# yangt1013/SPEINet

Measured on AMD Instinct MI355X. Metric: deblurred 720p frames/sec, higher is better.
Workload: dtype f16 (correlation top2)

## Files before the change

### speinet_amd/csrc/conv32_ws16.hip

```cpp
#include "common.h"

namespace {

constexpr int C = 32, KS = 5, PAD = 2, NTAP = KS * KS;
constexpr int TH = 16, TW = 32;
constexpr int IH = TH + KS - 1, IW = TW + KS - 1;
constexpr int PITCH = 2 * C + 16;
constexpr int SLAB = IH * IW * PITCH;
constexpr int NTHR = 256, RT = 4;

struct WsParams {
    const void* a;
    const void* wfrag;
    const float* bias;
    void* out;
    int H, W, batch, act;
    int tiles_x, tiles_y, total;
    long long* stamps;
};

__device__ __forceinline__ void mfma_aw(f32x16& acc, const lpv<_Float16>::x8& w, const lpv<_Float16>::x8& b) {
    asm volatile("v_mfma_f32_32x32x16_f16 %0, %1, %2, %0" : "+v"(acc) : "a"(w), "v"(b));
}
__device__ __forceinline__ void mfma_aw(f32x16& acc, const lpv<__bf16>::x8& w, const lpv<__bf16>::x8& b) {
    asm volatile("v_mfma_f32_32x32x16_bf16 %0, %1, %2, %0" : "+v"(acc) : "a"(w), "v"(b));
}

template <typename TA> struct Chunk { static constexpr int CPP = sizeof(TA) == 4 ? 8 : 4; };

template <typename LP, typename TA, typename TO>
__global__ __launch_bounds__(NTHR, 1) void conv32_ws_kernel(const WsParams p) {
    typedef typename lpv<LP>::x8 lp8;
    typedef typename lpv<LP>::x4 lp4;
    constexpr int CPP = Chunk<TA>::CPP;
    constexpr int NCH = IH * IW * CPP;
    constexpr int NIT = (NCH + NTHR - 1) / NTHR;
    constexpr int NPH = sizeof(TA) == 4 ? 2 : 1;
    constexpr int NITH = (NIT + NPH - 1) / NPH;
    extern __shared__ __attribute__((aligned(16))) unsigned char smem[];

    const int tid = threadIdx.x, lane = tid & 63, wave = tid >> 6;
    const int fr = lane & 31, fk = lane >> 5;

    lp8 wreg[NTAP][2];
    {
        const LP* wp = static_cast<const LP*>(p.wfrag) + lane * 8;
#pragma unroll
        for (int t = 0; t < NTAP; ++t)
#pragma unroll
            for (int s = 0; s < 2; ++s) wreg[t][s] = *reinterpret_cast<const lp8*>(wp + (t * 2 + s) * 512);
    }
    float biasv[16];
#pragma unroll
    for (int r = 0; r < 16; ++r) biasv[r] = p.bias ? p.bias[8 * (r >> 2) + 4 * fk + (r & 3)] : 0.f;

    typedef u32x4 stage_t;
    stage_t sreg[NITH];
    const size_t map_elems = (size_t)p.H * p.W * C;
    const int per_map = p.tiles_x * p.tiles_y;

    auto tile_origin = [&](int t, int& b, int& oy0, int& ox0) {
        b = t / per_map;
        const int r = t - b * per_map;
        const int ty = r / p.tiles_x;
        oy0 = ty * TH;
        ox0 = (r - ty * p.tiles_x) * TW;
    };
    constexpr int PPI = NTHR / CPP, E = 16 / (int)sizeof(TA);
    const int p0 = tid / CPP, sub = tid - p0 * CPP;
    const int iy0 = p0 / IW, ix0 = p0 - iy0 * IW;
    const int lds0 = p0 * PITCH + sub * (sizeof(TA) == 4 ? 8 : 16);
    auto advance = [](int& iy, int& ix) {
        ix += PPI % IW;
        iy += PPI / IW;
        if (ix >= IW) { ix -= IW; ++iy; }
    };
    auto load_slab = [&](int t, int ph) {
        int b, oy0, ox0;
        tile_origin(t, b, oy0, ox0);
        const TA* base = static_cast<const TA*>(p.a) + (size_t)b * map_elems + sub * E;
        int iy = iy0, ix = ix0;
#pragma unroll
        for (int it = 0; it < NIT; ++it) {
            if (it >= ph * NITH && it < (ph + 1) * NITH) {
                const int iyc = min(iy, IH - 1);
                const int gy = min(max(oy0 - PAD + iyc, 0), p.H - 1), gx = min(max(ox0 - PAD + ix, 0), p.W - 1);
                sreg[it - ph * NITH] = *reinterpret_cast<const stage_t*>(base + (gy * p.W + gx) * C);
            }
            advance(iy, ix);
        }
    };
    auto store_slab = [&](int t, int buf, int ph, int lo, int hi) {
        int b, oy0, ox0;
        tile_origin(t, b, oy0, ox0);
        unsigned char* sl = smem + buf * SLAB + lds0;
        int iy = iy0, ix = ix0;
#pragma unroll
        for (int it = 0; it < NIT; ++it) {
            if (it >= ph * NITH + lo && it < ph * NITH + hi && it < (ph + 1) * NITH && iy < IH) {
                const int j = it - ph * NITH;
                const bool ok = ((unsigned)(oy0 - PAD + iy) < (unsigned)p.H) & ((unsigned)(ox0 - PAD + ix) < (unsigned)p.W);
                if constexpr (sizeof(TA) == 4) {
                    const f32x4 v = __builtin_bit_cast(f32x4, sreg[j]);
                    lp4 h = to_lp4<LP>(v);
                    if (!ok) h = lp4{(LP)0.f, (LP)0.f, (LP)0.f, (LP)0.f};
                    *reinterpret_cast<lp4*>(sl + it * PPI * PITCH) = h;
                } else {
                    *reinterpret_cast<stage_t*>(sl + it * PPI * PITCH) = ok ? sreg[j] : stage_t{0u, 0u, 0u, 0u};
                }
            }
            advance(iy, ix);
        }
    };

    int t = blockIdx.x;
    if (t >= p.total) return;
#pragma unroll
    for (int ph = 0; ph < NPH; ++ph) {
        load_slab(t, ph);
        store_slab(t, 0, ph, 0, NITH);
    }
    lds_barrier();

    int boff[RT];
#pragma unroll
    for (int i = 0; i < RT; ++i) boff[i] = ((wave * RT + i) * IW + fr) * PITCH + fk * 16;

    int buf = 0;
    for (; t < p.total; t += gridDim.x, buf ^= 1) {
        const int tn = t + gridDim.x;
        const bool more = tn < p.total;
        const int tl = more ? tn : t;
        const bool st_ = t == (int)blockIdx.x + (int)gridDim.x;
        if (st_) SPEI_STAMP(p.stamps, 0);
        load_slab(tl, 0);
        if (st_) SPEI_STAMP(p.stamps, 1);
        __builtin_amdgcn_sched_barrier(0);

        const unsigned char* sl = smem + buf * SLAB;
        f32x16 acc[RT];
#pragma unroll
        for (int i = 0; i < RT; ++i)
#pragma unroll
            for (int r = 0; r < 16; ++r) acc[i][r] = biasv[r];
        lp8 bq[3][RT];
        auto step_off = [](int step) { const int tap = step >> 1; return ((tap / KS) * IW + (tap % KS)) * PITCH + (step & 1) * 32; };
#pragma unroll
        for (int d = 0; d < 2; ++d)
#pragma unroll
            for (int i = 0; i < RT; ++i) bq[d][i] = *reinterpret_cast<const lp8*>(sl + boff[i] + step_off(d));
#pragma unroll
        for (int step = 0; step < NTAP * 2; ++step) {
            const int tap = step >> 1, s2 = step & 1;
            if (step + 2 < NTAP * 2) {
#pragma unroll
                for (int i = 0; i < RT; ++i) bq[(step + 2) % 3][i] = *reinterpret_cast<const lp8*>(sl + boff[i] + step_off(step + 2));
            }
#pragma unroll
            for (int i = 0; i < RT; ++i) mfma_aw(acc[i], wreg[tap][s2], bq[step % 3][i]);
            if (NPH == 2 && step == NTAP) {
                store_slab(tl, buf ^ 1, 0, 0, NITH);
                load_slab(tl, 1);
            }
            if (NPH == 1 && step >= NTAP && ((step - NTAP) & 1) == 0 && (step - NTAP) / 2 < NITH)
                store_slab(tl, buf ^ 1, 0, (step - NTAP) / 2, (step - NTAP) / 2 + 1);
        }

        if (st_) SPEI_STAMP(p.stamps, 2);
        {
            int b, oy0, ox0;
            tile_origin(t, b, oy0, ox0);
            TO* ob = static_cast<TO*>(p.out) + (size_t)b * map_elems;
            const int ox = ox0 + fr;
#pragma unroll
            for (int i = 0; i < RT; ++i) {
                const int oy = oy0 + wave * RT + i;
                if (oy < p.H && ox < p.W) {
                    TO* o = ob + ((size_t)oy * p.W + ox) * C + 4 * fk;
#pragma unroll
                    for (int g = 0; g < 4; ++g) {
                        f32x4 v = {acc[i][4 * g], acc[i][4 * g + 1], acc[i][4 * g + 2], acc[i][4 * g + 3]};
                        if (p.act == SPEI_ACT_RELU) v = f32x4{fmaxf(v[0], 0.f), fmaxf(v[1], 0.f), fmaxf(v[2], 0.f), fmaxf(v[3], 0.f)};
                        if constexpr (sizeof(TO) == 4) *reinterpret_cast<f32x4*>(o + 8 * g) = v;
                        else *reinterpret_cast<lp4*>(o + 8 * g) = to_lp4<LP>(v);
                    }
                }
            }
        }
        if (st_) SPEI_STAMP(p.stamps, 3);
        if (NPH == 2) store_slab(tl, buf ^ 1, 1, 0, NITH);
        else store_slab(tl, buf ^ 1, 0, (NTAP + 1) / 2, NITH);
        if (st_) SPEI_STAMP(p.stamps, 4);
        lds_barrier();
        if (st_) SPEI_STAMP(p.stamps, 5);
    }
}

template <typename LP>
int launch_ws(const WsParams& p, int a16, int o16, hipStream_t st) {
    const size_t lds = 2 * (size_t)SLAB;
    const int cus = spei_num_cus();
    const dim3 grid(p.total < cus ? p.total : cus);
    if (a16 && o16) {
        ensure_dyn_lds<&conv32_ws_kernel<LP, LP, LP>>(lds);
        hipLaunchKernelGGL((conv32_ws_kernel<LP, LP, LP>), grid, dim3(NTHR), lds, st, p);
    } else if (!a16 && o16) {
        ensure_dyn_lds<&conv32_ws_kernel<LP, float, LP>>(lds);
        hipLaunchKernelGGL((conv32_ws_kernel<LP, float, LP>), grid, dim3(NTHR), lds, st, p);
    } else if (a16 && !o16) {
        ensure_dyn_lds<&conv32_ws_kernel<LP, LP, float>>(lds);
        hipLaunchKernelGGL((conv32_ws_kernel<LP, LP, float>), grid, dim3(NTHR), lds, st, p);
    } else {
        ensure_dyn_lds<&conv32_ws_kernel<LP, float, float>>(lds);
        hipLaunchKernelGGL((conv32_ws_kernel<LP, float, float>), grid, dim3(NTHR), lds, st, p);
    }
    return 0;
}

}

extern "C" int spei_conv32_ws16(int fmt, const void* a, int a_fmt, const void* wfrag, const float* bias, void* out, int out_fmt, int batch,
                                int H, int W, int act, spei_stream_t stream) {
    SPEI_REQUIRE(a && wfrag && out, "spei_conv32_ws16: null pointer");
    SPEI_REQUIRE((fmt == SPEI_BF16 || fmt == SPEI_F16) && (a_fmt == SPEI_F32 || a_fmt == fmt) && (out_fmt == SPEI_F32 || out_fmt == fmt),
                 "spei_conv32_ws16: fmt=%d a_fmt=%d out_fmt=%d", fmt, a_fmt, out_fmt);
    SPEI_REQUIRE(batch >= 1 && H > 0 && W > 0 && (int64_t)batch * cdiv(H, TH) * cdiv(W, TW) < (1ll << 30) && (int64_t)H * W < (1ll << 26),
                 "spei_conv32_ws16: batch=%d of %dx%d", batch, H, W);
    SPEI_REQUIRE(act == SPEI_ACT_NONE || act == SPEI_ACT_RELU, "spei_conv32_ws16: act=%d", act);
    SPEI_REQUIRE(((uintptr_t)a | (uintptr_t)wfrag | (uintptr_t)out) % 16 == 0 && a != out, "spei_conv32_ws16: 16-byte alignment, out must not be the input");
    WsParams p;
    p.a = a; p.wfrag = wfrag; p.bias = bias; p.out = out; p.H = H; p.W = W; p.batch = batch; p.act = act;
    p.tiles_x = cdiv(W, TW); p.tiles_y = cdiv(H, TH); p.total = batch * p.tiles_x * p.tiles_y;
    p.stamps = spei_stamp_buffer();
    hipStream_t st = (hipStream_t)stream;
    const int a16 = a_fmt != SPEI_F32, o16 = out_fmt != SPEI_F32;
    const int rc = fmt == SPEI_F16 ? launch_ws<_Float16>(p, a16, o16, st) : launch_ws<__bf16>(p, a16, o16, st);
    if (rc) return rc;
    SPEI_CHECK_LAUNCH("spei_conv32_ws16");
    return 0;
}
```

Baseline: 41.63.

## Software-pipeline conv32 tile loop: split accumulators, overlap epilogue and slab staging

Restructures the persistent 5x5 conv kernel so each tile is computed as two halves with separate accumulator pairs. The epilogue stores for one half, the bias reinit, and the chunked global loads and LDS stores for the next slab are interleaved step by step into the MFMA stream of the other half. The epilogue of the last tile is deferred past the loop. It also deepens the LDS operand prefetch ring and forces two staging phases for f16 input. This aims to hide store and load latency behind matrix work, in exchange for more register pressure, rigid sched_barrier ordering, and added s_nop hazards.

After: 41.81 (median of 6 runs). Within noise of the previous version (+0.4%).

```diff
diff --git a/speinet_amd/csrc/conv32_ws16.hip b/speinet_amd/csrc/conv32_ws16.hip
--- a/speinet_amd/csrc/conv32_ws16.hip
+++ b/speinet_amd/csrc/conv32_ws16.hip
@@ -8,6 +8,8 @@
 constexpr int PITCH = 2 * C + 16;
 constexpr int SLAB = IH * IW * PITCH;
 constexpr int NTHR = 256, RT = 4;
+constexpr int NSTEP = NTAP * 2;
+constexpr int EPI0 = 14, BIAS0 = EPI0 + 8;
 
 struct WsParams {
     const void* a;
@@ -19,11 +21,27 @@
     long long* stamps;
 };
 
+struct Origin { int b, oy0, ox0; };
+
 __device__ __forceinline__ void mfma_aw(f32x16& acc, const lpv<_Float16>::x8& w, const lpv<_Float16>::x8& b) {
     asm volatile("v_mfma_f32_32x32x16_f16 %0, %1, %2, %0" : "+v"(acc) : "a"(w), "v"(b));
 }
 __device__ __forceinline__ void mfma_aw(f32x16& acc, const lpv<__bf16>::x8& w, const lpv<__bf16>::x8& b) {
     asm volatile("v_mfma_f32_32x32x16_bf16 %0, %1, %2, %0" : "+v"(acc) : "a"(w), "v"(b));
+}
+
+template <int I, int N, typename F>
+__device__ __forceinline__ void static_for(F&& f) {
+    if constexpr (I < N) {
+        f(std::integral_constant<int, I>{});
+        static_for<I + 1, N>(f);
+    }
+}
+
+template <typename LP8>
+__device__ __forceinline__ void mfma_aw_first(f32x16& acc, const LP8& w, const LP8& b) {
+    asm volatile("s_nop 7" : "+v"(acc));
+    mfma_aw(acc, w, b);
 }
 
 template <typename TA> struct Chunk { static constexpr int CPP = sizeof(TA) == 4 ? 8 : 4; };
@@ -35,8 +53,10 @@
     constexpr int CPP = Chunk<TA>::CPP;
     constexpr int NCH = IH * IW * CPP;
     constexpr int NIT = (NCH + NTHR - 1) / NTHR;
-    constexpr int NPH = sizeof(TA) == 4 ? 2 : 1;
+    constexpr int NPH = 2;
     constexpr int NITH = (NIT + NPH - 1) / NPH;
+    constexpr int NRING = sizeof(TA) == 4 ? 4 : 6, AHEAD = NRING - 1;
+    static_assert(1 + NITH <= EPI0 && BIAS0 + 4 <= NSTEP - NITH, "a half's slices must not share a step");
     extern __shared__ __attribute__((aligned(16))) unsigned char smem[];
 
     const int tid = threadIdx.x, lane = tid & 63, wave = tid >> 6;
@@ -59,12 +79,14 @@
     const size_t map_elems = (size_t)p.H * p.W * C;
     const int per_map = p.tiles_x * p.tiles_y;
 
-    auto tile_origin = [&](int t, int& b, int& oy0, int& ox0) {
-        b = t / per_map;
-        const int r = t - b * per_map;
+    auto tile_origin = [&](int t) {
+        Origin o;
+        o.b = t / per_map;
+        const int r = t - o.b * per_map;
         const int ty = r / p.tiles_x;
-        oy0 = ty * TH;
-        ox0 = (r - ty * p.tiles_x) * TW;
+        o.oy0 = ty * TH;
+        o.ox0 = (r - ty * p.tiles_x) * TW;
+        return o;
     };
     constexpr int PPI = NTHR / CPP, E = 16 / (int)sizeof(TA);
     const int p0 = tid / CPP, sub = tid - p0 * CPP;
@@ -75,125 +97,141 @@
         iy += PPI / IW;
         if (ix >= IW) { ix -= IW; ++iy; }
     };
-    auto load_slab = [&](int t, int ph) {
-        int b, oy0, ox0;
-        tile_origin(t, b, oy0, ox0);
-        const TA* base = static_cast<const TA*>(p.a) + (size_t)b * map_elems + sub * E;
-        int iy = iy0, ix = ix0;
-#pragma unroll
-        for (int it = 0; it < NIT; ++it) {
-            if (it >= ph * NITH && it < (ph + 1) * NITH) {
-                const int iyc = min(iy, IH - 1);
-                const int gy = min(max(oy0 - PAD + iyc, 0), p.H - 1), gx = min(max(ox0 - PAD + ix, 0), p.W - 1);
-                sreg[it - ph * NITH] = *reinterpret_cast<const stage_t*>(base + (gy * p.W + gx) * C);
+    Origin stg;
+    int liy, lix, siy, six;
+    const TA* lbase;
+    auto load_chunk = [&](int it) {
+        if (it == 0) {
+            liy = iy0, lix = ix0;
+            lbase = static_cast<const TA*>(p.a) + (size_t)stg.b * map_elems + sub * E;
+        }
+        const int iyc = min(liy, IH - 1);
+        const int gy = min(max(stg.oy0 - PAD + iyc, 0), p.H - 1), gx = min(max(stg.ox0 - PAD + lix, 0), p.W - 1);
+        sreg[it % NITH] = *reinterpret_cast<const stage_t*>(lbase + (gy * p.W + gx) * C);
+        advance(liy, lix);
+    };
+    auto store_chunk = [&](int it, int buf) {
+        if (it == 0) siy = iy0, six = ix0;
+        if (siy < IH) {
+            unsigned char* d = smem + buf * SLAB + lds0 + it * PPI * PITCH;
+            const bool ok = ((unsigned)(stg.oy0 - PAD + siy) < (unsigned)p.H) & ((unsigned)(stg.ox0 - PAD + six) < (unsigned)p.W);
+            if constexpr (sizeof(TA) == 4) {
+                const f32x4 v = __builtin_bit_cast(f32x4, sreg[it % NITH]);
+                lp4 h = to_lp4<LP>(v);
+                if (!ok) h = lp4{(LP)0.f, (LP)0.f, (LP)0.f, (LP)0.f};
+                *reinterpret_cast<lp4*>(d) = h;
+            } else {
+                *reinterpret_cast<stage_t*>(d) = ok ? sreg[it % NITH] : stage_t{0u, 0u, 0u, 0u};
             }
-            advance(iy, ix);
-        }
-    };
-    auto store_slab = [&](int t, int buf, int ph, int lo, int hi) {
-        int b, oy0, ox0;
-        tile_origin(t, b, oy0, ox0);
-        unsigned char* sl = smem + buf * SLAB + lds0;
-        int iy = iy0, ix = ix0;
-#pragma unroll
-        for (int it = 0; it < NIT; ++it) {
-            if (it >= ph * NITH + lo && it < ph * NITH + hi && it < (ph + 1) * NITH && iy < IH) {
-                const int j = it - ph * NITH;
-                const bool ok = ((unsigned)(oy0 - PAD + iy) < (unsigned)p.H) & ((unsigned)(ox0 - PAD + ix) < (unsigned)p.W);
-                if constexpr (sizeof(TA) == 4) {
-                    const f32x4 v = __builtin_bit_cast(f32x4, sreg[j]);
-                    lp4 h = to_lp4<LP>(v);
-                    if (!ok) h = lp4{(LP)0.f, (LP)0.f, (LP)0.f, (LP)0.f};
-                    *reinterpret_cast<lp4*>(sl + it * PPI * PITCH) = h;
-                } else {
-                    *reinterpret_cast<stage_t*>(sl + it * PPI * PITCH) = ok ? sreg[j] : stage_t{0u, 0u, 0u, 0u};
-                }
-            }
-            advance(iy, ix);
-        }
+        }
+        advance(siy, six);
+    };
+    TO* eptr;
+    bool eok;
+    auto epilogue = [&](const f32x16 (&acc)[2], int pair, int s, const Origin& o, bool valid) {
+        const int i = s >> 2, g = s & 3;
+        if (g == 0) {
+            const int oy = o.oy0 + wave * RT + 2 * pair + i, ox = o.ox0 + fr;
+            eok = valid && oy < p.H && ox < p.W;
+            eptr = static_cast<TO*>(p.out) + (size_t)o.b * map_elems + ((size_t)oy * p.W + ox) * C + 4 * fk;
+        }
+        if (eok) {
+            f32x4 v = {acc[i][4 * g], acc[i][4 * g + 1], acc[i][4 * g + 2], acc[i][4 * g + 3]};
+            if (p.act == SPEI_ACT_RELU) v = f32x4{fmaxf(v[0], 0.f), fmaxf(v[1], 0.f), fmaxf(v[2], 0.f), fmaxf(v[3], 0.f)};
+            if constexpr (sizeof(TO) == 4) *reinterpret_cast<f32x4*>(eptr + 8 * g) = v;
+            else *reinterpret_cast<lp4*>(eptr + 8 * g) = to_lp4<LP>(v);
+        }
+    };
+    auto to_bias = [&](f32x16 (&acc)[2], int s) {
+#pragma unroll
+        for (int r = 0; r < 8; ++r) acc[s >> 1][8 * (s & 1) + r] = biasv[8 * (s & 1) + r];
     };
 
     int t = blockIdx.x;
     if (t >= p.total) return;
+    Origin cur = tile_origin(t), prev = cur;
+    stg = cur;
 #pragma unroll
     for (int ph = 0; ph < NPH; ++ph) {
-        load_slab(t, ph);
-        store_slab(t, 0, ph, 0, NITH);
+#pragma unroll
+        for (int it = ph * NITH; it < NIT && it < (ph + 1) * NITH; ++it) load_chunk(it);
+#pragma unroll
+        for (int it = ph * NITH; it < NIT && it < (ph + 1) * NITH; ++it) store_chunk(it, 0);
     }
     lds_barrier();
 
     int boff[RT];
 #pragma unroll
     for (int i = 0; i < RT; ++i) boff[i] = ((wave * RT + i) * IW + fr) * PITCH + fk * 16;
+
+    f32x16 acc0[2], acc1[2];
+#pragma unroll
+    for (int s = 0; s < 4; ++s) to_bias(acc0, s), to_bias(acc1, s);
+    bool have_prev = false;
 
     int buf = 0;
     for (; t < p.total; t += gridDim.x, buf ^= 1) {
         const int tn = t + gridDim.x;
-        const bool more = tn < p.total;
-        const int tl = more ? tn : t;
+        const int tl = tn < p.total ? tn : t;
         const bool st_ = t == (int)blockIdx.x + (int)gridDim.x;
-        if (st_) SPEI_STAMP(p.stamps, 0);
-        load_slab(tl, 0);
-        if (st_) SPEI_STAMP(p.stamps, 1);
+        if (st_) { SPEI_STAMP(p.stamps, 0); SPEI_STAMP_CLK(p.stamps, 8); }
         __builtin_amdgcn_sched_barrier(0);
 
         const unsigned char* sl = smem + buf * SLAB;
-        f32x16 acc[RT];
-#pragma unroll
-        for (int i = 0; i < RT; ++i)
-#pragma unroll
-            for (int r = 0; r < 16; ++r) acc[i][r] = biasv[r];
-        lp8 bq[3][RT];
-        auto step_off = [](int step) { const int tap = step >> 1; return ((tap / KS) * IW + (tap % KS)) * PITCH + (step & 1) * 32; };
-#pragma unroll
-        for (int d = 0; d < 2; ++d)
-#pragma unroll
-            for (int i = 0; i < RT; ++i) bq[d][i] = *reinterpret_cast<const lp8*>(sl + boff[i] + step_off(d));
-#pragma unroll
-        for (int step = 0; step < NTAP * 2; ++step) {
-            const int tap = step >> 1, s2 = step & 1;
-            if (step + 2 < NTAP * 2) {
-#pragma unroll
-                for (int i = 0; i < RT; ++i) bq[(step + 2) % 3][i] = *reinterpret_cast<const lp8*>(sl + boff[i] + step_off(step + 2));
+        lp8 bq[NRING][2];
+        auto fetch = [&](int q) {
+            const int h = q / NSTEP, tap = (q % NSTEP) >> 1;
+            const int off = ((tap / KS) * IW + (tap % KS)) * PITCH + (q & 1) * 32;
+#pragma unroll
+            for (int i = 0; i < 2; ++i) bq[q % NRING][i] = *reinterpret_cast<const lp8*>(sl + boff[2 * h + i] + off);
+        };
+#pragma unroll
+        for (int q = 0; q < AHEAD; ++q) fetch(q);
+
+        static_for<0, NSTEP>([&](auto sc) {
+            constexpr int s = decltype(sc)::value;
+            fetch(s + AHEAD);
+            __builtin_amdgcn_sched_barrier(0);
+#pragma unroll
+            for (int i = 0; i < 2; ++i) {
+                if constexpr (s == 0) mfma_aw_first(acc0[i], wreg[0][0], bq[0][i]);
+                else mfma_aw(acc0[i], wreg[s >> 1][s & 1], bq[s % NRING][i]);
             }
-#pragma unroll
-            for (int i = 0; i < RT; ++i) mfma_aw(acc[i], wreg[tap][s2], bq[step % 3][i]);
-            if (NPH == 2 && step == NTAP) {
-                store_slab(tl, buf ^ 1, 0, 0, NITH);
-                load_slab(tl, 1);
+            if constexpr (s == 0) stg = tile_origin(tl);
+            if constexpr (s >= 1 && s <= NITH) load_chunk(s - 1);
+            if constexpr (s >= EPI0 && s < EPI0 + 8) epilogue(acc1, 1, s - EPI0, prev, have_prev);
+            if constexpr (s >= BIAS0 && s < BIAS0 + 4) to_bias(acc1, s - BIAS0);
+            if constexpr (s >= NSTEP - NITH) store_chunk(s - (NSTEP - NITH), buf ^ 1);
+            __builtin_amdgcn_sched_barrier(0);
+        });
+        if (st_) { SPEI_STAMP(p.stamps, 1); SPEI_STAMP_CLK(p.stamps, 9); }
+        static_for<0, NSTEP>([&](auto sc) {
+            constexpr int s = decltype(sc)::value;
+            if constexpr (s + AHEAD < NSTEP) fetch(NSTEP + s + AHEAD);
+            __builtin_amdgcn_sched_barrier(0);
+#pragma unroll
+            for (int i = 0; i < 2; ++i) {
+                if constexpr (s == 0) mfma_aw_first(acc1[i], wreg[0][0], bq[NSTEP % NRING][i]);
+                else mfma_aw(acc1[i], wreg[s >> 1][s & 1], bq[(NSTEP + s) % NRING][i]);
             }
-            if (NPH == 1 && step >= NTAP && ((step - NTAP) & 1) == 0 && (step - NTAP) / 2 < NITH)
-                store_slab(tl, buf ^ 1, 0, (step - NTAP) / 2, (step - NTAP) / 2 + 1);
-        }
-
-        if (st_) SPEI_STAMP(p.stamps, 2);
-        {
-            int b, oy0, ox0;
-            tile_origin(t, b, oy0, ox0);
-            TO* ob = static_cast<TO*>(p.out) + (size_t)b * map_elems;
-            const int ox = ox0 + fr;
-#pragma unroll
-            for (int i = 0; i < RT; ++i) {
-                const int oy = oy0 + wave * RT + i;
-                if (oy < p.H && ox < p.W) {
-                    TO* o = ob + ((size_t)oy * p.W + ox) * C + 4 * fk;
-#pragma unroll
-                    for (int g = 0; g < 4; ++g) {
-                        f32x4 v = {acc[i][4 * g], acc[i][4 * g + 1], acc[i][4 * g + 2], acc[i][4 * g + 3]};
-                        if (p.act == SPEI_ACT_RELU) v = f32x4{fmaxf(v[0], 0.f), fmaxf(v[1], 0.f), fmaxf(v[2], 0.f), fmaxf(v[3], 0.f)};
-                        if constexpr (sizeof(TO) == 4) *reinterpret_cast<f32x4*>(o + 8 * g) = v;
-                        else *reinterpret_cast<lp4*>(o + 8 * g) = to_lp4<LP>(v);
-                    }
-                }
-            }
-        }
-        if (st_) SPEI_STAMP(p.stamps, 3);
-        if (NPH == 2) store_slab(tl, buf ^ 1, 1, 0, NITH);
-        else store_slab(tl, buf ^ 1, 0, (NTAP + 1) / 2, NITH);
-        if (st_) SPEI_STAMP(p.stamps, 4);
+            if constexpr (s >= 1 && s <= NIT - NITH) load_chunk(NITH + s - 1);
+            if constexpr (s >= EPI0 && s < EPI0 + 8) epilogue(acc0, 0, s - EPI0, cur, true);
+            if constexpr (s >= BIAS0 && s < BIAS0 + 4) to_bias(acc0, s - BIAS0);
+            if constexpr (s >= NSTEP - (NIT - NITH)) store_chunk(NITH + s - (NSTEP - (NIT - NITH)), buf ^ 1);
+            __builtin_amdgcn_sched_barrier(0);
+        });
+        if (st_) { SPEI_STAMP(p.stamps, 2); SPEI_STAMP_CLK(p.stamps, 10); }
         lds_barrier();
-        if (st_) SPEI_STAMP(p.stamps, 5);
-    }
+        if (st_) { SPEI_STAMP(p.stamps, 3); SPEI_STAMP_CLK(p.stamps, 11); }
+        prev = cur;
+        cur = stg;
+        have_prev = true;
+    }
+    SPEI_STAMP(p.stamps, 6); SPEI_STAMP_CLK(p.stamps, 14);
+    asm volatile("s_nop 7\n\ts_nop 7\n\ts_nop 7" : "+v"(acc1[0]), "+v"(acc1[1]));
+#pragma unroll
+    for (int s = 0; s < 8; ++s) epilogue(acc1, 1, s, prev, true);
+    SPEI_STAMP(p.stamps, 7); SPEI_STAMP_CLK(p.stamps, 15);
 }
 
 template <typename LP>
```
